# si220/Forest-SLAM

Measured on AMD Instinct MI355X. Metric: stereo frames/sec (extract+match+local-BA) at 600p, 1/8 MI355X; ATE RMSE, higher is better.
Workload: dtype mixed: u8/u16 integer (FAST, BRIEF, Hamming, SGM), f32 (ORB angle/Harris, back-projection), f64 (PnP, BA incl. its Schur GEMM on f64 MFMA)

## Files before the change

forest-slam_amd/csrc/capi.cpp:

```cpp
#include <cstddef>
#include <cstdio>
#include <cstring>

#include "fvo_internal.h"

int fvo_fail(fvo_ctx* ctx, const std::string& msg) {
  if (ctx) ctx->err = msg;
  return -1;
}

hipEvent_t fvo_event(fvo_ctx* ctx) {
  if (!ctx->tpool.empty()) {
    hipEvent_t e = ctx->tpool.back();
    ctx->tpool.pop_back();
    return e;
  }
  hipEvent_t e = nullptr;
  (void)hipEventCreate(&e);
  return e;
}

static_assert(sizeof(fvo_config) == 31 * 4, "fvo_config layout changed: bump FVO_ABI_VERSION");
static_assert(offsetof(fvo_config, scale_factor) == 16 && offsetof(fvo_config, sgbm_max_batch) == 104 &&
                  offsetof(fvo_config, sgbm_handoff_us) == 120,
// ... 36 lines not shown
  c->num_disparities = 6 * 16;
  c->block_size = 7;
  c->P1 = 8 * 7 * 7;
  c->P2 = 32 * 7 * 7;
  c->disp12_max_diff = 0;
  c->pre_filter_cap = 0;
  c->uniqueness_ratio = 0;
  c->sgbm_stripes = 4;
  c->kp_capacity = 0;
  c->stages = FVO_STAGE_ALL;
  c->ba_window = 10;
  c->ba_max_landmarks = 4096;
  c->ba_max_obs = 32768;
  c->sgbm_max_batch = 0;
  c->sgbm_mode = FVO_SGBM_CLASSIC;
  c->sgbm_lanes = 0;
  c->sgbm_cols = 0;
  c->sgbm_handoff_us = 0;
}

static void release(fvo_ctx* c) {
  void* ptrs[] = {c->pyr,        c->blur,      c->score,     c->cand,     c->hel,
                  c->ncand,      c->nsel1,     c->nsel2,     c->koff,     c->scratch, c->fast_rec, c->rt.xofs,  c->rt.xc1,
                  c->rt.yofs,    c->rt.yc1,    c->umax,      c->bf_rowkey, c->bf_colkey, c->bf_knn, c->sg_ckpt,
                  c->sg_V,      c->sg_M,      c->sg_raw,    c->sg_hand,   c->sg_ctl,    c->pnp_hyp,  c->pnp_good,
                  c->pnp_sub,    c->rs_table, c->pnp_models, c->pnp_ws, c->pnp_state, c->pnp_plan, c->pnp_pts, c->ba_ws,
                  c->em_x, c->em_models, c->em_good, c->em_nmod, c->em_state, c->em_ws};
  for (void* p : ptrs)
    if (p) (void)hipFree(p);
  if (c->ba_s2) (void)hipStreamDestroy(c->ba_s2);

  if (c->ba_fork) (void)hipEventDestroy(c->ba_fork);
  if (c->ba_join) (void)hipEventDestroy(c->ba_join);
}

int fvo_create(int device, const fvo_config* cfg, fvo_ctx** out) {
  if (!cfg || !out) return -1;
  *out = nullptr;
  fvo_ctx* c = new fvo_ctx();
  c->device = device;
  c->cfg = *cfg;
  auto bail = [&](int rc) {
    std::fprintf(stderr, "fvo_create: %s\n", c->err.c_str());
    release(c);
    delete c;
    return rc;
  };
// ... 359 lines not shown
```

forest-slam_amd/csrc/fvo_internal.h:

```cpp
#pragma once

#include <hip/hip_runtime.h>

#include <cstdint>
#include <string>
#include <vector>

#include "../../include/fvo.h"

#define FVO_MAX_LEVELS 12

struct OrbGeom {
  int nlevels;
  int w[FVO_MAX_LEVELS], h[FVO_MAX_LEVELS];
  float scale[FVO_MAX_LEVELS];
  int64_t off[FVO_MAX_LEVELS + 1];
  int row0[FVO_MAX_LEVELS + 1];
  int nfeat[FVO_MAX_LEVELS];
  int64_t cand_off[FVO_MAX_LEVELS + 1];
  int64_t total_px;
  int total_rows;
  int64_t cand_total;
};

// ... 22 lines not shown
struct fvo_ctx {
  int device = 0;
  uint64_t tmask = 0;
  std::vector<TimingRec> trecs;
  std::vector<hipEvent_t> tpool;
  fvo_config cfg{};
  OrbGeom g{};
  std::string err;
  int kp_cap = 0;
  int64_t ws_bytes = 0;
  uint8_t* pyr = nullptr;
  uint8_t* blur = nullptr;
  int orb_last_batch = 0;
  uint8_t* score = nullptr;
  uint32_t* cand = nullptr;
  uint64_t* hel = nullptr;
  int32_t* ncand = nullptr;
  int32_t* nsel1 = nullptr;
  int32_t* nsel2 = nullptr;
  int32_t* koff = nullptr;
  int32_t* scratch = nullptr;
  int64_t scratch_per = 0;
  ResizeTab rt{};
  int32_t* umax = nullptr;
  uint32_t* bf_rowkey = nullptr;
  uint32_t* bf_colkey = nullptr;
  uint32_t* bf_knn = nullptr;
  uint16_t* sg_V = nullptr;
  uint16_t* sg_M = nullptr;
  uint32_t* sg_ckpt = nullptr;
  int16_t* sg_raw = nullptr;
  uint64_t* sg_hand = nullptr;
  uint32_t* sg_ctl = nullptr;
  struct {
    bool valid = false;
    const void* matches = nullptr;
    const void* nmatch = nullptr;
    const void* stereo = nullptr;
    int nframes = 0, first_end = 0, nwin = 0, first_valid = 0;
  } ba_births;
  double* pnp_hyp = nullptr;
  int32_t* pnp_sub = nullptr;
  int16_t* rs_table = nullptr;
  int32_t rs_table_iters = 0;
  double* pnp_models = nullptr;
  double* pnp_ws = nullptr;
// ... 119 lines not shown
```

forest-slam_amd/csrc/orb.hip:

```cpp
#include <cmath>
#include <cstring>

#include "fvo_device.h"
#include "orb_pattern.inc"

namespace {

struct OrbDev {
  int nlevels, total_rows;
  int row0[FVO_MAX_LEVELS + 1];
  int w[FVO_MAX_LEVELS], h[FVO_MAX_LEVELS];
  long long off[FVO_MAX_LEVELS + 1];
  long long cand_off[FVO_MAX_LEVELS + 1];
  float scale[FVO_MAX_LEVELS];
  int nfeat[FVO_MAX_LEVELS];
  int tile0[FVO_MAX_LEVELS + 1];
  int ntx[FVO_MAX_LEVELS];
  int btile0[FVO_MAX_LEVELS + 1];
  int bntx[FVO_MAX_LEVELS];
};
__constant__ int c_umax[20];
__constant__ signed char c_pattern[256 * 4];

constexpr int kSelThreads = 512;
constexpr int kSelCap1 = 10000, kSelCap2 = 4096;

// ... 68 lines not shown
    if (win8) {
      const uint64_t wa = window(sa), wb = window(sb);
#pragma unroll
      for (int i = 0; i < kResCols; ++i) {
        const int da = 8 * (oxa[i] - oxa[0]), db = 8 * (oxb[i] - oxa[0]);
        const uint32_t ha = cx0[i] * (uint32_t)((wa >> da) & 255u) + cx1[i] * (uint32_t)((wa >> db) & 255u);
        const uint32_t hb = cx0[i] * (uint32_t)((wb >> da) & 255u) + cx1[i] * (uint32_t)((wb >> db) & 255u);
        v[k][i] = (ha * cy0 + hb * cy1 + 32768u) >> 16;
      }
    } else {
#pragma unroll
      for (int i = 0; i < kResCols; ++i) {
        const uint32_t ha = cx0[i] * sa[oxa[i]] + cx1[i] * sa[oxb[i]], hb = cx0[i] * sb[oxa[i]] + cx1[i] * sb[oxb[i]];
        v[k][i] = (ha * cy0 + hb * cy1 + 32768u) >> 16;
      }
    }
  }
#pragma unroll
  for (int k = 0; k < kResRows; ++k) {
    const int y = xb.y * kResRows + k;
#pragma unroll
    for (int i = 0; i < kResCols; ++i)
      if (y < h && x0 + i < w) dst[(int64_t)y * w + x0 + i] = (uint8_t)(v[k][i] > 255u ? 255u : v[k][i]);
  }
}

__constant__ int c_cdx[16] = {0, 1, 2, 3, 3, 3, 2, 1, 0, -1, -2, -3, -3, -3, -2, -1};
__constant__ int c_cdy[16] = {3, 3, 2, 1, 0, -1, -2, -3, -3, -3, -2, -1, 0, 1, 2, 3};

constexpr int kTW = 64, kTH = 32, kFT = 256;
static_assert(kTH <= 64 && kFT >= 2 * kTH && kFT % 64 == 0, "FAST tile shape");
constexpr int kRecKeep = 0, kRecPre = 8 * kTH, kRecSc = kRecPre + 2 * kTH;
constexpr int kTRec = kRecSc + kTH * kTW / 2;

constexpr int kFW = kTW + 2, kFH = kTH + 2;
constexpr int kPG = (kFW + 3) / 4;
constexpr int kIC = 4, kIW = kTW + 12, kIH = kTH + 8;

typedef unsigned short u16x2 __attribute__((ext_vector_type(2)));
__device__ __forceinline__ u16x2 as_u16x2(uint32_t v) { return __builtin_bit_cast(u16x2, v); }
__device__ __forceinline__ uint32_t as_u32(u16x2 v) { return __builtin_bit_cast(uint32_t, v); }
__device__ __forceinline__ u16x2 bytes02(uint32_t v) { return as_u16x2(__builtin_amdgcn_perm(0u, v, 0x0c020c00u)); }
__device__ __forceinline__ u16x2 bytes13(uint32_t v) { return as_u16x2(__builtin_amdgcn_perm(0u, v, 0x0c030c01u)); }

__device__ __forceinline__ u16x2 two_of_four(u16x2 a, u16x2 b, u16x2 c, u16x2 d) {
  const u16x2 lab = __builtin_elementwise_min(a, b), hab = __builtin_elementwise_max(a, b);
// ... 569 lines not shown
  counts[b] = s <= cap ? s : -s;
}

__device__ __forceinline__ float fast_atan2_deg(float y, float x) {
  const float k = (float)(180 / 3.14159265358979323846);
  const float p1 = 0.9997878412794807f * k, p3 = -0.3258083974640975f * k, p5 = 0.1555786518463281f * k,
              p7 = -0.04432655554792128f * k;
  const float eps = (float)2.220446049250313080847e-16;
  float ax = fabsf(x), ay = fabsf(y), a, c, c2;
  if (ax >= ay) {
    c = ay / (ax + eps);
    c2 = c * c;
    a = (((p7 * c2 + p5) * c2 + p3) * c2 + p1) * c;
  } else {
    c = ax / (ay + eps);
    c2 = c * c;
    a = 90.f - (((p7 * c2 + p5) * c2 + p3) * c2 + p1) * c;
  }
  if (x < 0) a = 180.f - a;
  if (y < 0) a = 360.f - a;
  return a;
}

__global__ void k_angle(const OrbDev G, const uint8_t* __restrict__ pyr, const uint64_t* __restrict__ hel,
                        const int32_t* __restrict__ nsel2, const int32_t* __restrict__ koff, float* __restrict__ kp,
                        int64_t total, int64_t cand_total, int nlevels, int cap, int patch) {
  const XcdBlock xb = xcd_block();
  int l = xb.y, b = xb.z;
  int n = nsel2[b * nlevels + l];
  int base = koff[b * (nlevels + 1) + l];
  int wpb = blockDim.x >> 6, lane = wave_lane();
  const uint8_t* im = pyr + b * total + G.off[l];
  int w = G.w[l];
  const uint64_t* hin = hel + b * cand_total + G.cand_off[l];
  const int half = patch / 2;
  for (int i = xb.x * wpb + (threadIdx.x >> 6); i < n; i += gridDim.x * wpb) {
    if (base + i >= cap) break;
    uint64_t e = hin[i];
    int x0 = (int)(e & 0xFFF), y0 = (int)((e >> 12) & 0xFFF);
    float resp = __uint_as_float((uint32_t)(e >> 32));
    const uint8_t* c = im + (int64_t)y0 * w + x0;
    int m10 = 0, m01 = 0;
    int u = lane - half;
    if (lane <= 2 * half) {
      m10 += u * c[u];
      if (half == 15) {
        int vp[15], vm[15];
#pragma unroll
        for (int v = 1; v <= 15; ++v) {
          vp[v - 1] = c[u + v * w];
          vm[v - 1] = c[u - v * w];
        }
#pragma unroll
        for (int v = 1; v <= 15; ++v) {
          const int d = c_umax[v];
          if (u >= -d && u <= d) {
            m01 += v * (vp[v - 1] - vm[v - 1]);
            m10 += u * (vp[v - 1] + vm[v - 1]);
          }
        }
      } else {
        for (int v = 1; v <= half; ++v) {
          int d = c_umax[v];
          if (u >= -d && u <= d) {
            int vp = c[u + v * w], vm = c[u - v * w];
            m01 += v * (vp - vm);
            m10 += u * (vp + vm);
          }
        }
      }
    }
    m10 = wave_sum(m10);
    m01 = wave_sum(m01);
    if (lane == 0) {
      float s = G.scale[l];
      float* o = kp + ((int64_t)b * cap + base + i) * FVO_KP_STRIDE;
      o[0] = (float)x0 * s;
      o[1] = (float)y0 * s;
      o[2] = patch * s;
      o[3] = fast_atan2_deg((float)m01, (float)m10);
      o[4] = resp;
      o[5] = (float)l;
      o[6] = -1.f;
      o[7] = 0.f;
    }
  }
}

__constant__ int c_gk[7] = {18, 34, 49, 55, 49, 34, 18};

__device__ __forceinline__ int reflect101(int i, int n) {
  i = i < 0 ? -i : i;
  return i >= n ? 2 * n - 2 - i : i;
}

constexpr int kBW = 256, kBH = 32;

__device__ __forceinline__ int btile_level(const OrbDev& G, int t) {
  int l = 0;
#pragma unroll
  for (int k = 1; k < FVO_MAX_LEVELS; ++k)
    if (k < G.nlevels && t >= G.btile0[k]) l = k;
  return l;
}

__global__ __launch_bounds__(256) void k_blur(const OrbDev G, const uint8_t* __restrict__ pyr,
                                              uint8_t* __restrict__ blur, int64_t total) {
  constexpr int RW = kBW + 6, RH = kBH + 6;
  __shared__ uint8_t s_img[RH][RW + 2];
  const int b = blockIdx.y, t = blockIdx.x;
  const int l = btile_level(G, t);
// ... 14 lines not shown
  int win[7] = {0, 0, 0, 0, 0, 0, 0};
#pragma unroll
  for (int r = 0; r < RH; ++r) {
    int hs = 0;
#pragma unroll
    for (int k = 0; k < 7; ++k) hs += c_gk[k] * s_img[r][c + k];
#pragma unroll
    for (int j = 0; j < 6; ++j) win[j] = win[j + 1];
    win[6] = hs;
    if (r >= 6) {
      const int y = y0 + r - 6;
      int sv = 0;
#pragma unroll
      for (int j = 0; j < 7; ++j) sv += c_gk[j] * win[j];
      const int q = (sv + 32767 + ((sv >> 16) & 1)) >> 16;
      if (xin && y < h) out[(int64_t)y * w] = (uint8_t)min(q, 255);
    }
  }
}

constexpr int kBrR = 19, kBrP = 2 * kBrR + 1, kBrS = kBrP + 6;
constexpr int kBrSW = kBrS + 3, kBrPW = kBrP + 1;

__global__ __launch_bounds__(256, 4) void k_brief(const OrbDev G, const uint8_t* __restrict__ pyr,
                                               const float* __restrict__ kp, const int32_t* __restrict__ counts,
                                               uint8_t* __restrict__ desc, int64_t total, int cap) {
  __shared__ __attribute__((aligned(16))) uint8_t s_src[4][kBrS][kBrSW];
  __shared__ uint8_t s_blr[4][kBrP][kBrPW];
  const XcdBlock xb = xcd_block();
  const int b = xb.y;
  const int n = counts[b];
  if (n < 0) return;
  const int wpb = blockDim.x >> 6, lane = wave_lane(), wv = threadIdx.x >> 6;
  uint8_t(*src)[kBrSW] = s_src[wv];
  uint8_t(*blr)[kBrPW] = s_blr[wv];
  for (int j = xb.x * wpb + wv; j < n; j += gridDim.x * wpb) {
    const float* k = kp + ((int64_t)b * cap + j) * FVO_KP_STRIDE;
    const int l = (int)k[5];
    const float scale = 1.f / G.scale[l];
    float angle = k[3];
    angle *= (float)(3.14159265358979323846 / 180.f);
    const float a = (float)cos((double)angle), bb = (float)sin((double)angle);
    const int cy = (int)rintf(k[1] * scale), cx = (int)rintf(k[0] * scale);
    const int w = G.w[l], h = G.h[l];
    const uint8_t* im = pyr + b * total + G.off[l];
    const int sx0 = cx - kBrR - 3, sy0 = cy - kBrR - 3;
    if (sx0 >= 0 && sy0 >= 0 && sx0 + kBrS <= w && sy0 + kBrS <= h) {
      constexpr int kRW = kBrSW / 4, kN = kBrS * kRW, kIt = (kN + 63) / 64;
      const uint8_t* p0 = im + (int64_t)sy0 * w + sx0;
#pragma unroll
      for (int t = 0; t < kIt; ++t) {
        const int i = min(lane + 64 * t, kN - 1);
        const int r = i / kRW, q = i - r * kRW;
        const uintptr_t pa = reinterpret_cast<uintptr_t>(p0 + r * w + 4 * q);
        const uint32_t* a4 = reinterpret_cast<const uint32_t*>(pa & ~(uintptr_t)3);
        const uint32_t v = __builtin_amdgcn_alignbyte(a4[1], a4[0], (uint32_t)pa & 3u);
        if (lane + 64 * t < kN) reinterpret_cast<uint32_t*>(&src[r][0])[q] = v;
      }
    } else {
      constexpr int kBrN = kBrS * kBrS;
#pragma unroll 1
      for (int i = lane; i < kBrN; i += 64) {
        const int r = i / kBrS, c = i - r * kBrS;
        const int y = reflect101(min(sy0 + r, 2 * (h - 1)), h);
        const int x = reflect101(min(sx0 + c, 2 * (w - 1)), w);
        src[r][c] = im[(int64_t)y * w + x];
      }
    }
    __builtin_amdgcn_s_waitcnt(0);
    __builtin_amdgcn_wave_barrier();
    if (lane < kBrP) {
      const int c = lane;
      int win[7] = {0, 0, 0, 0, 0, 0, 0};
      const uint32_t sh = (uint32_t)c & 3u;
#pragma unroll 1
      for (int r0 = 0; r0 < kBrS; r0 += 7) {
#pragma unroll
        for (int t = 0; t < 7; ++t) {
          const int r = r0 + t;
          if (r < kBrS) {
            const uint32_t* rw = reinterpret_cast<const uint32_t*>(&src[r][0]) + (c >> 2);
            const uint32_t d0 = rw[0], d1 = rw[1], d2 = rw[2];
            win[t] = (int)__builtin_amdgcn_udot4(__builtin_amdgcn_alignbyte(d2, d1, sh), 0x00122231u,
                                                 __builtin_amdgcn_udot4(__builtin_amdgcn_alignbyte(d1, d0, sh),
                                                                        0x37312212u, 0u, false),
                                                 false);
            if (r >= 6) {
              int sv = 0;
#pragma unroll
              for (int q = 0; q < 7; ++q) sv += c_gk[q] * win[(t + 1 + q) % 7];
              const int v = (sv + 32767 + ((sv >> 16) & 1)) >> 16;
              blr[r - 6][c] = (uint8_t)min(v, 255);
            }
          }
        }
      }
    }
    __builtin_amdgcn_s_waitcnt(0);
    __builtin_amdgcn_wave_barrier();
    unsigned long long words[4];
#pragma unroll
    for (int q = 0; q < 4; ++q) {
      const int pi = q * 64 + lane;
      int v[2];
#pragma unroll
      for (int s2 = 0; s2 < 2; ++s2) {
        const float px = (float)c_pattern[pi * 4 + 2 * s2], py = (float)c_pattern[pi * 4 + 2 * s2 + 1];
        const float xx = px * a - py * bb;
        const float yy = px * bb + py * a;
        const int ix = (int)rintf(xx), iy = (int)rintf(yy);
        v[s2] = blr[iy + kBrR][ix + kBrR];
      }
      words[q] = __ballot(v[0] < v[1]);
    }
    if (lane < 4) {
      const unsigned long long wv4 = lane == 0 ? words[0] : lane == 1 ? words[1] : lane == 2 ? words[2] : words[3];
      reinterpret_cast<unsigned long long*>(desc + ((int64_t)b * cap + j) * FVO_DESC_BYTES)[lane] = wv4;
    }
    __builtin_amdgcn_wave_barrier();
  }
}

// ... 31 lines not shown
    int rw = std::max(g.w[l] - 2 * c.edge_threshold, 0), rh = std::max(g.h[l] - 2 * c.edge_threshold, 0);
    g.cand_off[l] = coff;
    coff += (int64_t)((rw + 1) / 2) * ((rh + 1) / 2) + 1;
  }
  g.off[c.nlevels] = off;
  g.row0[c.nlevels] = row;
  g.cand_off[c.nlevels] = coff;
  g.total_px = (off + 255) / 256 * 256;
  g.total_rows = row;
  g.cand_total = coff;
  {
    float factor = (float)(1.0 / sf);
    float nd = c.nfeatures * (1 - factor) / (1 - (float)std::pow((double)factor, (double)c.nlevels));
    int sum = 0;
    for (int l = 0; l < c.nlevels - 1; ++l) {
      g.nfeat[l] = cv_round_f(nd);
      sum += g.nfeat[l];
      nd *= factor;
    }
    g.nfeat[c.nlevels - 1] = std::max(c.nfeatures - sum, 0);
  }

  std::vector<int32_t> xo, xc, yo, yc;
  auto coeffs = [](int src, int dst, std::vector<int32_t>& ofs, std::vector<int32_t>& c1) {
    double inv_scale = (double)dst / (double)src;
    double scale = 1.0 / inv_scale;
    for (int d = 0; d < dst; ++d) {
      double fval = scale * ((double)d + 0.5) - 0.5;
      int ival = (int)std::floor(fval);
      if (ival >= 0 && src > 1) {
        if (ival < src - 1) {
          double frac = fval - (double)ival;
          ofs.push_back(ival);
          c1.push_back(frac < 0 ? 0 : (int)std::llrint(frac * 256.0));
        } else {
          ofs.push_back(-2);
          c1.push_back(0);
        }
      } else {
        ofs.push_back(-1);
        c1.push_back(0);
      }
    }
  };
  for (int l = 1; l < c.nlevels; ++l) {
    ctx->rt.xoff[l] = (int64_t)xo.size();
    coeffs(g.w[l - 1], g.w[l], xo, xc);
    ctx->rt.yoff[l] = (int64_t)yo.size();
    coeffs(g.h[l - 1], g.h[l], yo, yc);
  }
  if (xo.empty()) { xo.push_back(0); xc.push_back(0); yo.push_back(0); yc.push_back(0); }
  int rc = 0;
  if ((rc = fvo_alloc(ctx, &ctx->rt.xofs, xo.size())) || (rc = fvo_alloc(ctx, &ctx->rt.xc1, xc.size())) ||
      (rc = fvo_alloc(ctx, &ctx->rt.yofs, yo.size())) || (rc = fvo_alloc(ctx, &ctx->rt.yc1, yc.size())))
    return rc;
  FVO_HIP(ctx, hipMemcpy(ctx->rt.xofs, xo.data(), xo.size() * 4, hipMemcpyHostToDevice));
  FVO_HIP(ctx, hipMemcpy(ctx->rt.xc1, xc.data(), xc.size() * 4, hipMemcpyHostToDevice));
  FVO_HIP(ctx, hipMemcpy(ctx->rt.yofs, yo.data(), yo.size() * 4, hipMemcpyHostToDevice));
  FVO_HIP(ctx, hipMemcpy(ctx->rt.yc1, yc.data(), yc.size() * 4, hipMemcpyHostToDevice));

  int half = c.patch_size / 2;
  std::vector<int> umax(half + 2 > 20 ? half + 2 : 20, 0);
  int vmax = (int)std::floor(half * std::sqrt(2.f) / 2 + 1);
  int vmin = (int)std::ceil(half * std::sqrt(2.f) / 2);
  for (int v = 0; v <= vmax; ++v) umax[v] = (int)std::lrint(std::sqrt((double)half * half - v * v));
  for (int v = half, v0 = 0; v >= vmin; --v) {
    while (umax[v0] == umax[v0 + 1]) ++v0;
    umax[v] = v0;
    ++v0;
  }

  FVO_HIP(ctx, hipMemcpyToSymbol(HIP_SYMBOL(c_umax), umax.data(), sizeof(int) * 20));
  FVO_HIP(ctx, hipMemcpyToSymbol(HIP_SYMBOL(c_pattern), FVO_ORB_PATTERN, sizeof(FVO_ORB_PATTERN)));

  const int64_t B = c.max_batch;
  int64_t maxcand = 0;
  for (int l = 0; l < c.nlevels; ++l) maxcand = std::max<int64_t>(maxcand, g.cand_off[l + 1] - g.cand_off[l]);
  ctx->scratch_per = 2 * maxcand;
  if ((rc = fvo_alloc(ctx, &ctx->pyr, B * g.total_px)) ||
      (rc = fvo_alloc(ctx, &ctx->cand, B * g.cand_total)) ||
      (rc = fvo_alloc(ctx, &ctx->hel, B * g.cand_total)) || (rc = fvo_alloc(ctx, &ctx->ncand, B * c.nlevels)) ||
      (rc = fvo_alloc(ctx, &ctx->nsel1, B * c.nlevels)) || (rc = fvo_alloc(ctx, &ctx->nsel2, B * c.nlevels)) ||
      (rc = fvo_alloc(ctx, &ctx->koff, B * (c.nlevels + 1))) ||
      (rc = fvo_alloc(ctx, &ctx->scratch, B * c.nlevels * ctx->scratch_per)))
    return rc;
  if ((g.w[0] + kTW - 1) / kTW > 64) return fvo_fail(ctx, "ORB: image wider than 4096 px");
  if ((rc = fvo_alloc(ctx, &ctx->fast_rec, B * make_dev(g).tile0[g.nlevels] * kTRec))) return rc;
  return 0;
}

namespace {
OrbDev make_dev(const OrbGeom& g) {
  OrbDev G{};
// ... 16 lines not shown
    bt += G.bntx[l] * ((g.h[l] + kBH - 1) / kBH);
  }
  G.btile0[g.nlevels] = bt;
  G.row0[g.nlevels] = g.row0[g.nlevels];
  G.off[g.nlevels] = g.off[g.nlevels];
  G.cand_off[g.nlevels] = g.cand_off[g.nlevels];
  G.tile0[g.nlevels] = t;
  return G;
}
}

int orb_run(fvo_ctx* ctx, const uint8_t* images, int batch, int64_t image_stride, int pitch, float* kp, uint8_t* desc,
            int32_t* counts, int cap, hipStream_t s) {
  const fvo_config& c = ctx->cfg;
  const OrbGeom& g = ctx->g;
  const int L = g.nlevels;
  const int W = c.width, H = c.height;
  const int64_t total = g.total_px;
  const int thr = std::min(std::max(c.fast_threshold, 0), 255);
  const OrbDev G = make_dev(g);
  const int ntiles = G.tile0[L];
  const bool vec = ((uintptr_t)images & 15) == 0 && (image_stride & 15) == 0 && (pitch & 15) == 0 && (W & 15) == 0 &&
                   (total & 15) == 0;
  if (vec) {
    const int64_t n16 = (int64_t)batch * H * (W / 16);
    const int nblk = (int)std::min<int64_t>((n16 + 255) / 256, 4096);
    FVO_TIMED(ctx, KN_ORB_COPY, s, hipLaunchKernelGGL(k_copy_level0_v, dim3(nblk), dim3(256), 0, s,
                                                      reinterpret_cast<const uint4*>(images), image_stride / 16,
                                                      pitch / 16, reinterpret_cast<uint4*>(ctx->pyr), total / 16, W / 16,
                                                      H, batch));
  } else {
    FVO_TIMED(ctx, KN_ORB_COPY, s, hipLaunchKernelGGL(k_copy_level0, dim3((W + 255) / 256, H, batch), dim3(256), 0, s,
                                                      images, image_stride, pitch, ctx->pyr, total, W, H));
  }
  for (int l = 1; l < L; ++l)
    FVO_TIMED(ctx, KN_ORB_RESIZE, s, hipLaunchKernelGGL(k_resize, dim3((g.w[l] + 256 * kResCols - 1) / (256 * kResCols), (g.h[l] + kResRows - 1) / kResRows, batch), dim3(256), 0, s, G, ctx->pyr, total, l,
                       ctx->rt.xofs + ctx->rt.xoff[l], ctx->rt.xc1 + ctx->rt.xoff[l], ctx->rt.yofs + ctx->rt.yoff[l],
                       ctx->rt.yc1 + ctx->rt.yoff[l]));
  FVO_TIMED(ctx, KN_ORB_FAST, s, hipLaunchKernelGGL(k_fast_nms<false>, dim3(ntiles, batch), dim3(kFT), 0, s, G, ctx->pyr,
                     nullptr, ctx->fast_rec, total, thr, c.edge_threshold, ntiles));
  FVO_TIMED(ctx, KN_ORB_SELECT1, s, hipLaunchKernelGGL(HIP_KERNEL_NAME(k_select<ElemFast, kSelCap1, true>), dim3(batch, L),
                     dim3(kSelThreads), 0, s, G, ctx->fast_rec, ntiles, c.edge_threshold, ctx->cand, ctx->ncand,
                     ctx->nsel1, ctx->scratch, ctx->scratch_per, g.cand_total, L, 2));
  FVO_TIMED(ctx, KN_ORB_HARRIS, s, hipLaunchKernelGGL(k_harris, dim3(32, L, batch), dim3(256), 0, s, G, ctx->pyr, ctx->cand, ctx->nsel1, ctx->hel, total,
                     g.cand_total, L));
  FVO_TIMED(ctx, KN_ORB_SELECT2, s, hipLaunchKernelGGL(HIP_KERNEL_NAME(k_select<ElemHarris, kSelCap2, false>), dim3(batch, L),
                     dim3(kSelThreads), 0, s, G, nullptr, ntiles, c.edge_threshold, ctx->hel, ctx->nsel1,
                     ctx->nsel2, ctx->scratch, ctx->scratch_per, g.cand_total, L, 1));
  FVO_TIMED(ctx, KN_ORB_OFFSETS, s, hipLaunchKernelGGL(k_offsets, dim3((batch + 63) / 64), dim3(64), 0, s, ctx->nsel2, ctx->koff, counts, batch, L, cap));
  FVO_TIMED(ctx, KN_ORB_ANGLE, s, hipLaunchKernelGGL(k_angle, dim3(16, L, batch), dim3(256), 0, s, G, ctx->pyr, ctx->hel, ctx->nsel2, ctx->koff, kp,
                     total, g.cand_total, L, cap, c.patch_size));
  FVO_TIMED(ctx, KN_ORB_BRIEF, s, hipLaunchKernelGGL(k_brief, dim3(64, batch), dim3(256), 0, s, G, ctx->pyr, kp, counts, desc, total, cap));
  ctx->orb_last_batch = batch;
  FVO_LAUNCH_CHECK(ctx);
  return 0;
}

int orb_blur_debug(fvo_ctx* ctx) {
  if (!ctx->pyr) return fvo_fail(ctx, "orb stage not enabled");
  const OrbGeom& g = ctx->g;
  if (!ctx->blur) {
    int rc = fvo_alloc(ctx, &ctx->blur, (int64_t)ctx->cfg.max_batch * g.total_px);
    if (rc) return rc;
  }
  if (ctx->orb_last_batch > 0) {
    const OrbDev G = make_dev(g);
    hipLaunchKernelGGL(k_blur, dim3(G.btile0[g.nlevels], ctx->orb_last_batch), dim3(256), 0, 0, G, ctx->pyr, ctx->blur,
                       g.total_px);
    FVO_LAUNCH_CHECK(ctx);
  }
  FVO_HIP(ctx, hipDeviceSynchronize());
  return 0;
}

int orb_score_debug(fvo_ctx* ctx) {
// ... 51 lines not shown
```

profiles/summarize.py:

```python
import csv
import glob
import os
import sys
from collections import defaultdict


def find(d, pat):
    f = glob.glob(os.path.join(d, "**", pat), recursive=True)
    return f[0] if f else None


def ours(name):
    return any(k in name for k in ("k_sg_", "k_bf_", "k_pnp", "k_backproject", "k_brief", "k_blur", "k_angle",
                                   "k_harris", "k_select", "k_nms", "k_fast", "k_resize", "k_copy_level0",
                                   "k_row_scan", "k_offsets", "k_ba_", "k_em_", "k_ing_", "k_gather",
                                   "k_mb_", "k_map_", "k_vx_", "rocprim"))


def short(name):
    import re
    m = re.search(r"\b(k_[a-z0-9_]+)(<[^>(]*>)?", name)
    return (m.group(1) + (m.group(2) or "")) if m else name


def main(trace, fetch, write, out, shape):
    os.makedirs(out, exist_ok=True)
    st = find(trace, "*kernel_stats.csv")
    if st:
        rows = list(csv.DictReader(open(st)))
        keep = [r for r in rows if ours(r["Name"])]
        with open(os.path.join(out, "kernel_stats.csv"), "w", newline="") as f:
            w = csv.DictWriter(f, fieldnames=list(rows[0].keys()) + ["shape"])
            w.writeheader()
            for r in keep:
                r["Name"] = short(r["Name"])
                r["shape"] = shape
                w.writerow(r)
# ... 23 lines not shown
```

Before: 5815.

## Fuse ORB pyramid build into banded LDS kernel and merge angle into BRIEF

Replaces the level-0 copy plus one resize launch per level with a single k_pyramid kernel. Each block owns a horizontal band and builds every pyramid level in double-buffered LDS, using a host-planned band/halo table, then writes the levels out. It also removes k_angle by computing the intensity-centroid moments from the patch already staged in LDS inside k_brief. This is meant to cut launches and repeated global reads of intermediate levels, at the cost of recomputing halo rows and a large dynamic LDS allocation that may lower occupancy.

```diff
diff --git a/forest-slam_amd/csrc/capi.cpp b/forest-slam_amd/csrc/capi.cpp
--- a/forest-slam_amd/csrc/capi.cpp
+++ b/forest-slam_amd/csrc/capi.cpp
@@ -82,7 +82,7 @@
 static void release(fvo_ctx* c) {
   void* ptrs[] = {c->pyr,        c->blur,      c->score,     c->cand,     c->hel,
                   c->ncand,      c->nsel1,     c->nsel2,     c->koff,     c->scratch, c->fast_rec, c->rt.xofs,  c->rt.xc1,
-                  c->rt.yofs,    c->rt.yc1,    c->umax,      c->bf_rowkey, c->bf_colkey, c->bf_knn, c->sg_ckpt,
+                  c->rt.yofs,    c->rt.yc1,    c->orb_bands, c->umax,      c->bf_rowkey, c->bf_colkey, c->bf_knn, c->sg_ckpt,
                   c->sg_V,      c->sg_M,      c->sg_raw,    c->sg_hand,   c->sg_ctl,    c->pnp_hyp,  c->pnp_good,
                   c->pnp_sub,    c->rs_table, c->pnp_models, c->pnp_ws, c->pnp_state, c->pnp_plan, c->pnp_pts, c->ba_ws,
                   c->em_x, c->em_models, c->em_good, c->em_nmod, c->em_state, c->em_ws};
diff --git a/forest-slam_amd/csrc/fvo_internal.h b/forest-slam_amd/csrc/fvo_internal.h
--- a/forest-slam_amd/csrc/fvo_internal.h
+++ b/forest-slam_amd/csrc/fvo_internal.h
@@ -68,6 +68,9 @@
   int32_t* scratch = nullptr;
   int64_t scratch_per = 0;
   ResizeTab rt{};
+  int32_t* orb_bands = nullptr;
+  int orb_nbands = 0;
+  int orb_lds = 0, orb_lds_even = 0;
   int32_t* umax = nullptr;
   uint32_t* bf_rowkey = nullptr;
   uint32_t* bf_colkey = nullptr;
diff --git a/forest-slam_amd/csrc/orb.hip b/forest-slam_amd/csrc/orb.hip
--- a/forest-slam_amd/csrc/orb.hip
+++ b/forest-slam_amd/csrc/orb.hip
@@ -2,6 +2,7 @@
 #include <cstring>
 
 #include "fvo_device.h"
+#include "orb_bands.h"
 #include "orb_pattern.inc"
 
 namespace {
@@ -116,6 +117,187 @@
 #pragma unroll
     for (int i = 0; i < kResCols; ++i)
       if (y < h && x0 + i < w) dst[(int64_t)y * w + x0 + i] = (uint8_t)(v[k][i] > 255u ? 255u : v[k][i]);
+  }
+}
+
+constexpr int kPyrT = 512;
+constexpr int kPyrLds = kOrbBandLds;
+
+struct PyrTabs {
+  int xoff[FVO_MAX_LEVELS], yoff[FVO_MAX_LEVELS];
+};
+
+template <class D4, class B1>
+__device__ __forceinline__ void store_row(uint8_t* __restrict__ dst, int w, int lane, D4 dword_at, B1 byte_at) {
+  const int head = min((int)((4u - ((uint32_t)reinterpret_cast<uintptr_t>(dst) & 3u)) & 3u), w);
+  const int nd = (w - head) >> 2;
+  if (lane < head) dst[lane] = byte_at(lane);
+  uint32_t* d4 = reinterpret_cast<uint32_t*>(dst + head);
+  for (int k = lane; k < nd; k += 64) d4[k] = dword_at(head + 4 * k);
+  const int t0 = head + 4 * nd;
+  if (lane < w - t0) dst[t0 + lane] = byte_at(t0 + lane);
+}
+
+template <bool IMG>
+__device__ __forceinline__ void pyr_level(const uint8_t* src, int64_t spitch, int srow0, int sw, int sh, uint8_t* dst,
+                                          int dpitch, int c0, int c1, int w, const int32_t* __restrict__ xofs,
+                                          const int32_t* __restrict__ xc1, const int32_t* __restrict__ yofs,
+                                          const int32_t* __restrict__ yc1) {
+  const int ncg = dpitch / kResCols, nrg = (c1 - c0 + kResRows - 1) / kResRows;
+  const int cpb = min(ncg, kPyrT), nrl = kPyrT / cpb;
+  const int rl = (int)threadIdx.x / cpb, cl = (int)threadIdx.x - rl * cpb;
+  if (rl >= nrl || rl >= nrg) return;
+  auto ytab = [&](int rg, int* oy, uint32_t* cy) {
+#pragma unroll
+    for (int k = 0; k < kResRows; ++k) {
+      const int y = min(c0 + rg * kResRows + k, c1 - 1);
+      oy[k] = yofs[y];
+      cy[k] = (uint32_t)yc1[y];
+    }
+  };
+  int oy[kResRows];
+  uint32_t cy[kResRows];
+  ytab(rl, oy, cy);
+  for (int cg = cl; cg < ncg; cg += cpb) {
+    const int x0 = cg * kResCols;
+    int oxa[kResCols], oxb[kResCols];
+    uint32_t cx0[kResCols], cx1[kResCols];
+#pragma unroll
+    for (int i = 0; i < kResCols; ++i) {
+      const int ox = xofs[min(x0 + i, w - 1)];
+      oxa[i] = ox >= 0 ? ox : (ox == -1 ? 0 : sw - 1);
+      oxb[i] = ox >= 0 ? ox + 1 : oxa[i];
+      cx1[i] = ox >= 0 ? (uint32_t)xc1[min(x0 + i, w - 1)] : 0u;
+      cx0[i] = 256u - cx1[i];
+    }
+    const int span = oxb[kResCols - 1] - oxa[0];
+    const bool win8 = span <= 7;
+    auto window = [&](const uint8_t* row) -> uint64_t {
+      uint32_t sft, w0, w1, w2;
+      if (IMG) {
+        const uintptr_t pa = reinterpret_cast<uintptr_t>(row + oxa[0]);
+        const uint32_t* q = reinterpret_cast<const uint32_t*>(pa & ~(uintptr_t)3);
+        sft = (uint32_t)(pa & 3);
+        w0 = q[0];
+        w1 = q[(int)sft + span >= 4 ? 1 : 0];
+        w2 = q[(int)sft + span >= 8 ? 2 : 0];
+      } else {
+        const uint32_t* q = reinterpret_cast<const uint32_t*>(row) + (oxa[0] >> 2);
+        sft = (uint32_t)oxa[0] & 3u;
+        w0 = q[0], w1 = q[1], w2 = q[2];
+      }
+      return ((uint64_t)__builtin_amdgcn_alignbyte(w2, w1, sft) << 32) | __builtin_amdgcn_alignbyte(w1, w0, sft);
+    };
+    for (int rg = rl; rg < nrg; rg += nrl) {
+      int oyn[kResRows];
+      uint32_t cyn[kResRows];
+      ytab(min(rg + nrl, nrg - 1), oyn, cyn);
+      uint32_t v[kResRows][kResCols];
+#pragma unroll
+      for (int k = 0; k < kResRows; ++k) {
+        const int ra = oy[k] >= 0 ? oy[k] : (oy[k] == -1 ? 0 : sh - 1), rb = oy[k] >= 0 ? oy[k] + 1 : ra;
+        const uint32_t cy1 = oy[k] >= 0 ? cy[k] : 0u, cy0 = 256u - cy1;
+        const uint8_t* sa = src + (int64_t)(ra - srow0) * spitch;
+        const uint8_t* sb = src + (int64_t)(rb - srow0) * spitch;
+        if (win8) {
+          const uint64_t wa = window(sa), wb = window(sb);
+#pragma unroll
+          for (int i = 0; i < kResCols; ++i) {
+            const int da = 8 * (oxa[i] - oxa[0]), db = 8 * (oxb[i] - oxa[0]);
+            const uint32_t ha = cx0[i] * (uint32_t)((wa >> da) & 255u) + cx1[i] * (uint32_t)((wa >> db) & 255u);
+            const uint32_t hb = cx0[i] * (uint32_t)((wb >> da) & 255u) + cx1[i] * (uint32_t)((wb >> db) & 255u);
+            v[k][i] = (ha * cy0 + hb * cy1 + 32768u) >> 16;
+          }
+        } else {
+#pragma unroll
+          for (int i = 0; i < kResCols; ++i) {
+            const uint32_t ha = cx0[i] * sa[oxa[i]] + cx1[i] * sa[oxb[i]], hb = cx0[i] * sb[oxa[i]] + cx1[i] * sb[oxb[i]];
+            v[k][i] = (ha * cy0 + hb * cy1 + 32768u) >> 16;
+          }
+        }
+      }
+#pragma unroll
+      for (int k = 0; k < kResRows; ++k) {
+        const int y = c0 + rg * kResRows + k;
+        uint32_t p = 0;
+#pragma unroll
+        for (int i = 0; i < kResCols; ++i) p |= (v[k][i] > 255u ? 255u : v[k][i]) << (8 * i);
+        if (y < c1) *reinterpret_cast<uint32_t*>(dst + (y - c0) * dpitch + x0) = p;
+        oy[k] = oyn[k];
+        cy[k] = cyn[k];
+      }
+    }
+    if (cg + cpb < ncg) ytab(rl, oy, cy);
+  }
+}
+
+__global__ __launch_bounds__(kPyrT) void k_pyramid(const OrbDev G, const uint8_t* __restrict__ img, int64_t stride,
+                                                   int pitch, int vec, uint8_t* __restrict__ pyr, int64_t total,
+                                                   const int4* __restrict__ bands, int even_off,
+                                                   const int32_t* __restrict__ xofs, const int32_t* __restrict__ xc1,
+                                                   const int32_t* __restrict__ yofs, const int32_t* __restrict__ yc1,
+                                                   const PyrTabs T) {
+  extern __shared__ __attribute__((aligned(16))) uint8_t s_pyr[];
+  const int b = blockIdx.y, lane = wave_lane(), wv = threadIdx.x >> 6;
+  const int4* bt = bands + blockIdx.x * G.nlevels;
+  const uint8_t* im = img + b * stride;
+  uint8_t* out = pyr + b * total;
+  {
+    const int4 r = bt[0];
+    const int W = G.w[0];
+    if (vec) {
+      const int W16 = W >> 4, P16 = pitch >> 4, n = (r.y - r.x) * W16;
+      const uint4* s16 = reinterpret_cast<const uint4*>(im + (int64_t)r.x * pitch);
+      uint4* d16 = reinterpret_cast<uint4*>(out + (int64_t)r.x * W);
+      for (int i0 = threadIdx.x; i0 < n; i0 += 4 * kPyrT) {
+        uint4 t[4];
+#pragma unroll
+        for (int k = 0; k < 4; ++k) {
+          const int i = min(i0 + k * kPyrT, n - 1), y = i / W16;
+          t[k] = s16[(int64_t)y * P16 + (i - y * W16)];
+        }
+#pragma unroll
+        for (int k = 0; k < 4; ++k)
+          if (i0 + k * kPyrT < n) d16[i0 + k * kPyrT] = t[k];
+      }
+    } else {
+      for (int y = r.x + wv; y < r.y; y += kPyrT / 64) {
+        const uint8_t* srow = im + (int64_t)y * pitch;
+        store_row(
+            out + (int64_t)y * W, W, lane,
+            [&](int c) {
+              return (uint32_t)srow[c] | (uint32_t)srow[c + 1] << 8 | (uint32_t)srow[c + 2] << 16 |
+                     (uint32_t)srow[c + 3] << 24;
+            },
+            [&](int c) { return srow[c]; });
+      }
+    }
+  }
+  for (int l = 1; l < G.nlevels; ++l) {
+    const int4 r = bt[l];
+    const int w = G.w[l], dp = (w + 3) & ~3;
+    uint8_t* dst = s_pyr + ((l & 1) ? 0 : even_off);
+    if (r.w > r.z) {
+      if (l == 1) {
+        pyr_level<true>(im, pitch, 0, G.w[0], G.h[0], dst, dp, r.z, r.w, w, xofs + T.xoff[1], xc1 + T.xoff[1],
+                        yofs + T.yoff[1], yc1 + T.yoff[1]);
+      } else {
+        pyr_level<false>(s_pyr + ((l & 1) ? even_off : 0), (G.w[l - 1] + 3) & ~3, bt[l - 1].z, G.w[l - 1], G.h[l - 1],
+                         dst, dp, r.z, r.w, w, xofs + T.xoff[l], xc1 + T.xoff[l], yofs + T.yoff[l], yc1 + T.yoff[l]);
+      }
+    }
+    __syncthreads();
+    uint8_t* lout = out + G.off[l];
+    for (int y = r.x + wv; y < r.y; y += kPyrT / 64) {
+      const uint8_t* lrow = dst + (y - r.z) * dp;
+      store_row(
+          lout + (int64_t)y * w, w, lane,
+          [&](int c) {
+            const uint32_t* q = reinterpret_cast<const uint32_t*>(lrow) + (c >> 2);
+            return __builtin_amdgcn_alignbyte(q[1], q[0], (uint32_t)c & 3u);
+          },
+          [&](int c) { return lrow[c]; });
+    }
   }
 }
 
@@ -731,71 +913,6 @@
   return a;
 }
 
-__global__ void k_angle(const OrbDev G, const uint8_t* __restrict__ pyr, const uint64_t* __restrict__ hel,
-                        const int32_t* __restrict__ nsel2, const int32_t* __restrict__ koff, float* __restrict__ kp,
-                        int64_t total, int64_t cand_total, int nlevels, int cap, int patch) {
-  const XcdBlock xb = xcd_block();
-  int l = xb.y, b = xb.z;
-  int n = nsel2[b * nlevels + l];
-  int base = koff[b * (nlevels + 1) + l];
-  int wpb = blockDim.x >> 6, lane = wave_lane();
-  const uint8_t* im = pyr + b * total + G.off[l];
-  int w = G.w[l];
-  const uint64_t* hin = hel + b * cand_total + G.cand_off[l];
-  const int half = patch / 2;
-  for (int i = xb.x * wpb + (threadIdx.x >> 6); i < n; i += gridDim.x * wpb) {
-    if (base + i >= cap) break;
-    uint64_t e = hin[i];
-    int x0 = (int)(e & 0xFFF), y0 = (int)((e >> 12) & 0xFFF);
-    float resp = __uint_as_float((uint32_t)(e >> 32));
-    const uint8_t* c = im + (int64_t)y0 * w + x0;
-    int m10 = 0, m01 = 0;
-    int u = lane - half;
-    if (lane <= 2 * half) {
-      m10 += u * c[u];
-      if (half == 15) {
-        int vp[15], vm[15];
-#pragma unroll
-        for (int v = 1; v <= 15; ++v) {
-          vp[v - 1] = c[u + v * w];
-          vm[v - 1] = c[u - v * w];
-        }
-#pragma unroll
-        for (int v = 1; v <= 15; ++v) {
-          const int d = c_umax[v];
-          if (u >= -d && u <= d) {
-            m01 += v * (vp[v - 1] - vm[v - 1]);
-            m10 += u * (vp[v - 1] + vm[v - 1]);
-          }
-        }
-      } else {
-        for (int v = 1; v <= half; ++v) {
-          int d = c_umax[v];
-          if (u >= -d && u <= d) {
-            int vp = c[u + v * w], vm = c[u - v * w];
-            m01 += v * (vp - vm);
-            m10 += u * (vp + vm);
-          }
-        }
-      }
-    }
-    m10 = wave_sum(m10);
-    m01 = wave_sum(m01);
-    if (lane == 0) {
-      float s = G.scale[l];
-      float* o = kp + ((int64_t)b * cap + base + i) * FVO_KP_STRIDE;
-      o[0] = (float)x0 * s;
-      o[1] = (float)y0 * s;
-      o[2] = patch * s;
-      o[3] = fast_atan2_deg((float)m01, (float)m10);
-      o[4] = resp;
-      o[5] = (float)l;
-      o[6] = -1.f;
-      o[7] = 0.f;
-    }
-  }
-}
-
 __constant__ int c_gk[7] = {18, 34, 49, 55, 49, 34, 18};
 
 __device__ __forceinline__ int reflect101(int i, int n) {
@@ -856,26 +973,44 @@
 constexpr int kBrR = 19, kBrP = 2 * kBrR + 1, kBrS = kBrP + 6;
 constexpr int kBrSW = kBrS + 3, kBrPW = kBrP + 1;
 
+constexpr int kBrHalf = 15;
+
+__device__ __forceinline__ int wave_total(int v) {
+  v += __builtin_amdgcn_update_dpp(0, v, 0xB1, 0xF, 0xF, false);
+  v += __builtin_amdgcn_update_dpp(0, v, 0x4E, 0xF, 0xF, false);
+  v += __builtin_amdgcn_update_dpp(0, v, 0x141, 0xF, 0xF, false);
+  v += __builtin_amdgcn_update_dpp(0, v, 0x140, 0xF, 0xF, false);
+  return __builtin_amdgcn_readlane(v, 0) + __builtin_amdgcn_readlane(v, 16) + __builtin_amdgcn_readlane(v, 32) +
+         __builtin_amdgcn_readlane(v, 48);
+}
+
 __global__ __launch_bounds__(256, 4) void k_brief(const OrbDev G, const uint8_t* __restrict__ pyr,
-                                               const float* __restrict__ kp, const int32_t* __restrict__ counts,
-                                               uint8_t* __restrict__ desc, int64_t total, int cap) {
+                                               const uint64_t* __restrict__ hel, const int32_t* __restrict__ koff,
+                                               float* __restrict__ kp, const int32_t* __restrict__ counts,
+                                               uint8_t* __restrict__ desc, int64_t total, int64_t cand_total,
+                                               int nlevels, int cap) {
   __shared__ __attribute__((aligned(16))) uint8_t s_src[4][kBrS][kBrSW];
   __shared__ uint8_t s_blr[4][kBrP][kBrPW];
   const XcdBlock xb = xcd_block();
   const int b = xb.y;
-  const int n = counts[b];
-  if (n < 0) return;
+  const int cnt = counts[b];
+  const int n = min(cnt < 0 ? -cnt : cnt, cap);
   const int wpb = blockDim.x >> 6, lane = wave_lane(), wv = threadIdx.x >> 6;
   uint8_t(*src)[kBrSW] = s_src[wv];
   uint8_t(*blr)[kBrPW] = s_blr[wv];
+  const int32_t* ko = koff + b * (nlevels + 1);
+  const int mu = (lane & 31) - kBrHalf;
+  const int mvb = lane < 32 ? 1 : 8, mve = min(lane < 32 ? 7 : kBrHalf, c_umax[min(abs(mu), kBrHalf)]);
   for (int j = xb.x * wpb + wv; j < n; j += gridDim.x * wpb) {
-    const float* k = kp + ((int64_t)b * cap + j) * FVO_KP_STRIDE;
-    const int l = (int)k[5];
-    const float scale = 1.f / G.scale[l];
-    float angle = k[3];
-    angle *= (float)(3.14159265358979323846 / 180.f);
-    const float a = (float)cos((double)angle), bb = (float)sin((double)angle);
-    const int cy = (int)rintf(k[1] * scale), cx = (int)rintf(k[0] * scale);
+    int l = 0;
+    for (int q = 1; q < nlevels; ++q)
+      if (j >= ko[q]) l = q;
+    const uint64_t e = hel[b * cand_total + G.cand_off[l] + (j - ko[l])];
+    const int x0 = (int)(e & 0xFFF), y0 = (int)((e >> 12) & 0xFFF);
+    const float ls = G.scale[l];
+    const float kx = (float)x0 * ls, ky = (float)y0 * ls;
+    const float scale = 1.f / ls;
+    const int cy = (int)rintf(ky * scale), cx = (int)rintf(kx * scale);
     const int w = G.w[l], h = G.h[l];
     const uint8_t* im = pyr + b * total + G.off[l];
     const int sx0 = cx - kBrR - 3, sy0 = cy - kBrR - 3;
@@ -903,6 +1038,38 @@
     }
     __builtin_amdgcn_s_waitcnt(0);
     __builtin_amdgcn_wave_barrier();
+    int m10 = 0, m01 = 0;
+    if (mu <= kBrHalf) {
+      const int px = x0 - sx0 + mu, py = y0 - sy0;
+      if (lane < 32) m10 = mu * (int)src[py][px];
+#pragma unroll
+      for (int t = 0; t < 8; ++t) {
+        const int v = mvb + t;
+        if (v <= mve) {
+          const int vp = src[py + v][px], vm = src[py - v][px];
+          m01 += v * (vp - vm);
+          m10 += mu * (vp + vm);
+        }
+      }
+    }
+    m10 = wave_total(m10);
+    m01 = wave_total(m01);
+    float angle = fast_atan2_deg((float)m01, (float)m10);
+    if (lane == 0) {
+      float* o = kp + ((int64_t)b * cap + j) * FVO_KP_STRIDE;
+      o[0] = kx;
+      o[1] = ky;
+      o[2] = (2 * kBrHalf + 1) * ls;
+      o[3] = angle;
+      o[4] = __uint_as_float((uint32_t)(e >> 32));
+      o[5] = (float)l;
+      o[6] = -1.f;
+      o[7] = 0.f;
+    }
+    if (cnt < 0) {
+      __builtin_amdgcn_wave_barrier();
+      continue;
+    }
     if (lane < kBrP) {
       const int c = lane;
       int win[7] = {0, 0, 0, 0, 0, 0, 0};
@@ -932,6 +1099,8 @@
     }
     __builtin_amdgcn_s_waitcnt(0);
     __builtin_amdgcn_wave_barrier();
+    angle *= (float)(3.14159265358979323846 / 180.f);
+    const float a = (float)cos((double)angle), bb = (float)sin((double)angle);
     unsigned long long words[4];
 #pragma unroll
     for (int q = 0; q < 4; ++q) {
@@ -1009,32 +1178,11 @@
   }
 
   std::vector<int32_t> xo, xc, yo, yc;
-  auto coeffs = [](int src, int dst, std::vector<int32_t>& ofs, std::vector<int32_t>& c1) {
-    double inv_scale = (double)dst / (double)src;
-    double scale = 1.0 / inv_scale;
-    for (int d = 0; d < dst; ++d) {
-      double fval = scale * ((double)d + 0.5) - 0.5;
-      int ival = (int)std::floor(fval);
-      if (ival >= 0 && src > 1) {
-        if (ival < src - 1) {
-          double frac = fval - (double)ival;
-          ofs.push_back(ival);
-          c1.push_back(frac < 0 ? 0 : (int)std::llrint(frac * 256.0));
-        } else {
-          ofs.push_back(-2);
-          c1.push_back(0);
-        }
-      } else {
-        ofs.push_back(-1);
-        c1.push_back(0);
-      }
-    }
-  };
   for (int l = 1; l < c.nlevels; ++l) {
     ctx->rt.xoff[l] = (int64_t)xo.size();
-    coeffs(g.w[l - 1], g.w[l], xo, xc);
+    orb_resize_coeffs(g.w[l - 1], g.w[l], xo, xc);
     ctx->rt.yoff[l] = (int64_t)yo.size();
-    coeffs(g.h[l - 1], g.h[l], yo, yc);
+    orb_resize_coeffs(g.h[l - 1], g.h[l], yo, yc);
   }
   if (xo.empty()) { xo.push_back(0); xc.push_back(0); yo.push_back(0); yc.push_back(0); }
   int rc = 0;
@@ -1046,6 +1194,20 @@
   FVO_HIP(ctx, hipMemcpy(ctx->rt.yofs, yo.data(), yo.size() * 4, hipMemcpyHostToDevice));
   FVO_HIP(ctx, hipMemcpy(ctx->rt.yc1, yc.data(), yc.size() * 4, hipMemcpyHostToDevice));
 
+  {
+    const OrbBandPlan plan = orb_band_plan(c.nlevels, g.w, g.h, kPyrLds);
+    ctx->orb_nbands = plan.nbands;
+    ctx->orb_lds = plan.lds_bytes;
+    ctx->orb_lds_even = plan.buf_bytes[1];
+    if (plan.nbands > 0) {
+      std::vector<int32_t> bt;
+      for (const OrbBandRange& e : plan.r) bt.insert(bt.end(), {e.own0, e.own1, e.c0, e.c1});
+      if ((rc = fvo_alloc(ctx, &ctx->orb_bands, bt.size()))) return rc;
+      FVO_HIP(ctx, hipMemcpy(ctx->orb_bands, bt.data(), bt.size() * 4, hipMemcpyHostToDevice));
+      FVO_HIP(ctx, hipFuncSetAttribute((const void*)k_pyramid, hipFuncAttributeMaxDynamicSharedMemorySize, kPyrLds));
+    }
+  }
+
   int half = c.patch_size / 2;
   std::vector<int> umax(half + 2 > 20 ? half + 2 : 20, 0);
   int vmax = (int)std::floor(half * std::sqrt(2.f) / 2 + 1);
@@ -1056,6 +1218,10 @@
     umax[v] = v0;
     ++v0;
   }
+
+  for (int u = 0; u <= half; ++u)
+    for (int v = 0; v <= half; ++v)
+      if ((u <= umax[v]) != (v <= umax[u])) return fvo_fail(ctx, "ORB: the angle's circle is not symmetric");
 
   FVO_HIP(ctx, hipMemcpyToSymbol(HIP_SYMBOL(c_umax), umax.data(), sizeof(int) * 20));
   FVO_HIP(ctx, hipMemcpyToSymbol(HIP_SYMBOL(c_pattern), FVO_ORB_PATTERN, sizeof(FVO_ORB_PATTERN)));
@@ -1118,7 +1284,18 @@
   const int ntiles = G.tile0[L];
   const bool vec = ((uintptr_t)images & 15) == 0 && (image_stride & 15) == 0 && (pitch & 15) == 0 && (W & 15) == 0 &&
                    (total & 15) == 0;
-  if (vec) {
+  if (ctx->orb_nbands > 0) {
+    PyrTabs T{};
+    for (int l = 1; l < L; ++l) {
+      T.xoff[l] = (int)ctx->rt.xoff[l];
+      T.yoff[l] = (int)ctx->rt.yoff[l];
+    }
+    FVO_TIMED(ctx, KN_ORB_RESIZE, s,
+              hipLaunchKernelGGL(k_pyramid, dim3(ctx->orb_nbands, batch), dim3(kPyrT), (size_t)ctx->orb_lds, s, G, images,
+                                 image_stride, pitch, (int)vec, ctx->pyr, total,
+                                 reinterpret_cast<const int4*>(ctx->orb_bands), ctx->orb_lds_even, ctx->rt.xofs,
+                                 ctx->rt.xc1, ctx->rt.yofs, ctx->rt.yc1, T));
+  } else if (vec) {
     const int64_t n16 = (int64_t)batch * H * (W / 16);
     const int nblk = (int)std::min<int64_t>((n16 + 255) / 256, 4096);
     FVO_TIMED(ctx, KN_ORB_COPY, s, hipLaunchKernelGGL(k_copy_level0_v, dim3(nblk), dim3(256), 0, s,
@@ -1129,7 +1306,7 @@
     FVO_TIMED(ctx, KN_ORB_COPY, s, hipLaunchKernelGGL(k_copy_level0, dim3((W + 255) / 256, H, batch), dim3(256), 0, s,
                                                       images, image_stride, pitch, ctx->pyr, total, W, H));
   }
-  for (int l = 1; l < L; ++l)
+  for (int l = 1; l < L && ctx->orb_nbands == 0; ++l)
     FVO_TIMED(ctx, KN_ORB_RESIZE, s, hipLaunchKernelGGL(k_resize, dim3((g.w[l] + 256 * kResCols - 1) / (256 * kResCols), (g.h[l] + kResRows - 1) / kResRows, batch), dim3(256), 0, s, G, ctx->pyr, total, l,
                        ctx->rt.xofs + ctx->rt.xoff[l], ctx->rt.xc1 + ctx->rt.xoff[l], ctx->rt.yofs + ctx->rt.yoff[l],
                        ctx->rt.yc1 + ctx->rt.yoff[l]));
@@ -1144,9 +1321,8 @@
                      dim3(kSelThreads), 0, s, G, nullptr, ntiles, c.edge_threshold, ctx->hel, ctx->nsel1,
                      ctx->nsel2, ctx->scratch, ctx->scratch_per, g.cand_total, L, 1));
   FVO_TIMED(ctx, KN_ORB_OFFSETS, s, hipLaunchKernelGGL(k_offsets, dim3((batch + 63) / 64), dim3(64), 0, s, ctx->nsel2, ctx->koff, counts, batch, L, cap));
-  FVO_TIMED(ctx, KN_ORB_ANGLE, s, hipLaunchKernelGGL(k_angle, dim3(16, L, batch), dim3(256), 0, s, G, ctx->pyr, ctx->hel, ctx->nsel2, ctx->koff, kp,
-                     total, g.cand_total, L, cap, c.patch_size));
-  FVO_TIMED(ctx, KN_ORB_BRIEF, s, hipLaunchKernelGGL(k_brief, dim3(64, batch), dim3(256), 0, s, G, ctx->pyr, kp, counts, desc, total, cap));
+  FVO_TIMED(ctx, KN_ORB_BRIEF, s, hipLaunchKernelGGL(k_brief, dim3(64, batch), dim3(256), 0, s, G, ctx->pyr, ctx->hel, ctx->koff, kp, counts,
+                     desc, total, g.cand_total, L, cap));
   ctx->orb_last_batch = batch;
   FVO_LAUNCH_CHECK(ctx);
   return 0;
diff --git a/forest-slam_amd/csrc/orb_bands.h b/forest-slam_amd/csrc/orb_bands.h
--- /dev/null
+++ b/forest-slam_amd/csrc/orb_bands.h
@@ -0,0 +1,106 @@
+#pragma once
+
+#include <algorithm>
+#include <cmath>
+#include <cstdint>
+#include <vector>
+
+inline void orb_resize_coeffs(int src, int dst, std::vector<int32_t>& ofs, std::vector<int32_t>& c1) {
+  double inv_scale = (double)dst / (double)src;
+  double scale = 1.0 / inv_scale;
+  for (int d = 0; d < dst; ++d) {
+    double fval = scale * ((double)d + 0.5) - 0.5;
+    int ival = (int)std::floor(fval);
+    if (ival >= 0 && src > 1) {
+      if (ival < src - 1) {
+        double frac = fval - (double)ival;
+        ofs.push_back(ival);
+        c1.push_back(frac < 0 ? 0 : (int)std::llrint(frac * 256.0));
+      } else {
+        ofs.push_back(-2);
+        c1.push_back(0);
+      }
+    } else {
+      ofs.push_back(-1);
+      c1.push_back(0);
+    }
+  }
+}
+
+inline void orb_src_rows(int ofs, int src_h, int* ra, int* rb) {
+  *ra = ofs >= 0 ? ofs : (ofs == -1 ? 0 : src_h - 1);
+  *rb = ofs >= 0 ? ofs + 1 : *ra;
+}
+
+struct OrbBandRange {
+  int own0, own1;
+  int c0, c1;
+};
+
+constexpr int kOrbBandLds = 80 * 1024;
+constexpr int kOrbBandPad = 16;
+constexpr int kOrbBandMinRows = 8;
+constexpr int kOrbBandMaxRows = 64;
+
+inline int orb_band_stride(int w) { return (w + 3) / 4 * 4; }
+
+struct OrbBandPlan {
+  int nbands = 0;
+  int lds_bytes = 0, buf_bytes[2] = {0, 0};
+  std::vector<OrbBandRange> r;
+};
+
+inline std::vector<OrbBandRange> orb_band_ranges(int nlevels, const int* h, const std::vector<int32_t>* yofs,
+                                                 int nbands) {
+  std::vector<OrbBandRange> r((size_t)nbands * nlevels);
+  for (int k = 0; k < nbands; ++k) {
+    OrbBandRange* b = &r[(size_t)k * nlevels];
+    for (int l = nlevels - 1; l >= 0; --l) {
+      b[l].own0 = (int)((int64_t)k * h[l] / nbands);
+      b[l].own1 = (int)((int64_t)(k + 1) * h[l] / nbands);
+      int c0 = b[l].own0, c1 = b[l].own1;
+      if (l >= 1 && l + 1 < nlevels && b[l + 1].c1 > b[l + 1].c0) {
+        int ra, rb, s0, s1;
+        orb_src_rows(yofs[l + 1][b[l + 1].c0], h[l], &s0, &rb);
+        orb_src_rows(yofs[l + 1][b[l + 1].c1 - 1], h[l], &ra, &s1);
+        ++s1;
+        if (c1 > c0) { c0 = std::min(c0, s0); c1 = std::max(c1, s1); }
+        else { c0 = s0; c1 = s1; }
+      }
+      if (c1 <= c0) c0 = c1 = 0;
+      b[l].c0 = c0;
+      b[l].c1 = c1;
+    }
+  }
+  return r;
+}
+
+inline OrbBandPlan orb_band_plan(int nlevels, const int* w, const int* h, int budget) {
+  OrbBandPlan best;
+  if (nlevels < 2) return best;
+  std::vector<std::vector<int32_t>> yofs(nlevels);
+  for (int l = 1; l < nlevels; ++l) {
+    std::vector<int32_t> c1;
+    orb_resize_coeffs(h[l - 1], h[l], yofs[l], c1);
+  }
+  const int nmax = std::max(1, h[0] / kOrbBandMinRows);
+  for (int n = std::min(nmax, (h[0] + kOrbBandMaxRows - 1) / kOrbBandMaxRows); n <= nmax; ++n) {
+    std::vector<OrbBandRange> r = orb_band_ranges(nlevels, h, yofs.data(), n);
+    int64_t buf[2] = {0, 0};
+    for (int k = 0; k < n; ++k)
+      for (int l = 1; l < nlevels; ++l) {
+        const OrbBandRange& e = r[(size_t)k * nlevels + l];
+        buf[l & 1] = std::max<int64_t>(buf[l & 1], (int64_t)(e.c1 - e.c0) * orb_band_stride(w[l]));
+      }
+    const int64_t need = buf[0] + buf[1] + 2 * kOrbBandPad;
+    if (need <= budget) {
+      best.nbands = n;
+      best.buf_bytes[1] = (int)buf[1] + kOrbBandPad;
+      best.buf_bytes[0] = (int)buf[0] + kOrbBandPad;
+      best.lds_bytes = (int)need;
+      best.r = std::move(r);
+      return best;
+    }
+  }
+  return best;
+}
diff --git a/profiles/summarize.py b/profiles/summarize.py
--- a/profiles/summarize.py
+++ b/profiles/summarize.py
@@ -12,7 +12,7 @@
 
 def ours(name):
     return any(k in name for k in ("k_sg_", "k_bf_", "k_pnp", "k_backproject", "k_brief", "k_blur", "k_angle",
-                                   "k_harris", "k_select", "k_nms", "k_fast", "k_resize", "k_copy_level0",
+                                   "k_harris", "k_select", "k_nms", "k_fast", "k_resize", "k_copy_level0", "k_pyramid",
                                    "k_row_scan", "k_offsets", "k_ba_", "k_em_", "k_ing_", "k_gather",
                                    "k_mb_", "k_map_", "k_vx_", "rocprim"))
 
```

New measurement: 5815. Within noise of the previous version (-0.0%).
